# may-/joeys2t

Measured on AMD Instinct MI355X. Metric: audio frames/sec (train step, 80-mel, 15 s utt, bs32 per GPU), higher is better.
Workload: dtype bf16; 1 GPU; configs/librispeech_100h.yaml ASR train step on synthetic 16 kHz waveforms; global_batch=32, frames_per_utt=1498, encoder_len=375, lengths=fixed 15 s, vocab=5000, batch_multiplier=1, parallelism=dp1, launch=hipGraph replay

## Files before the change

### include/joeys2t_hip.h

```cpp
#ifndef JOEYS2T_HIP_H
#define JOEYS2T_HIP_H

#include <stdint.h>

#ifdef __cplusplus
extern "C" {
#endif

typedef void* js2t_stream;

enum { JS2T_F32 = 0, JS2T_BF16 = 1, JS2T_FP8_E4M3 = 2  };
enum { JS2T_ACT_NONE = 0, JS2T_ACT_RELU = 1, JS2T_ACT_GELU = 2, JS2T_ACT_SWISH = 3, JS2T_ACT_TANH = 4, JS2T_ACT_HARDSWISH = 5 };
enum { JS2T_OK = 0, JS2T_ERR_INVALID = -1, JS2T_ERR_LAUNCH = -2, JS2T_ERR_UNSUPPORTED = -3 };

int js2t_abi_version(void);
const char* js2t_last_error(void);

typedef struct js2t_gemm_desc {
  int32_t M, N, K;
  int32_t batch, batch_inner;
  int32_t dtype_ab, dtype_c;
  int32_t trans_a, trans_b;
  const void* A; int64_t lda, a_stride_o, a_stride_i;
  const void* B; int64_t ldb, b_stride_o, b_stride_i;
// ... 8 lines not shown
  uint32_t rng_stream;
  const void* residual;
  int64_t ldr;
  float res_scale;
  const void* gate;
  int64_t ldg;
  float gate_scale;
  float beta;
  int32_t conv, conv_tin, conv_tout, conv_c, conv_stride, conv_pad;
  int32_t split_k;
  float* a_rowsum;
  const float* ln_partial;
  float ln_eps;
  float* ln_mean;
  float* ln_rstd;
  float* rs_partial;
  uint8_t* c8;
  int64_t ldc8;
  float* c8_state;
  const float* c8_mul;
  float* c8_scale_out;
  float* fp8_state;
  const void* dot_src;
  int64_t ld_dot;
  float* dot_partial;
  float* sumsq_partial;
} js2t_gemm_desc;

int js2t_gemm(const js2t_gemm_desc* d, js2t_stream stream);
#define JS2T_GEMM_GROUP_MAX 32
int js2t_gemm_grouped(const js2t_gemm_desc* d, int32_t count, const void* const* A, const void* const* B, void* const* C,
                      float* const* a_rowsum, js2t_stream stream);
int64_t js2t_gemm_grouped_blocks(int32_t M, int32_t N, int32_t count);
void js2t_gemm_force_regstage(int on);
void js2t_gemm_force_w256(int on);
void js2t_gemm_p192_mode(int mode);
void js2t_gemm_wg256_mode(int mode);
void js2t_gemm_p192_ring(int nst);
void js2t_gemm_panel_mode(int mode);


int js2t_axpby(const void* x, float a, const void* y, float b, void* out, int64_t n, int dt, js2t_stream stream);

int js2t_cast(const void* src, int src_dt, void* dst, int dst_dt, int64_t n, js2t_stream stream);

int js2t_fold_ln_weights(const int64_t* table, int32_t n_entries, int32_t max_rows, js2t_stream stream);

int js2t_absmax(const void* x, int dt, int64_t n, float* out, js2t_stream stream);
int js2t_quantize_fp8(const void* x, int dt, void* y, int64_t n, const float* amax, const float* mul, float* scale_out,
                      js2t_stream stream);
int js2t_quantize_fp8_delayed(const void* x, int dt, void* y, int64_t n, float* state, const float* mul, float* scale_out,
                              js2t_stream stream);

int js2t_glu_fwd(const void* x, void* y, int64_t rows, int64_t C, int dt, js2t_stream stream);
int js2t_glu_bwd(const void* x, const void* dy, void* dx, int64_t rows, int64_t C, int dt, js2t_stream stream);
int js2t_glu_fwd_crop(const void* x, void* y, int64_t rows, int64_t C, int64_t T, const int64_t* valid_t, int dt, js2t_stream stream);
int js2t_glu_bwd_crop(const void* x, const void* dy, void* dx, int64_t rows, int64_t C, int64_t T, const int64_t* valid_t, int dt,
                      js2t_stream stream);

int js2t_transpose_groups(const void* src, void* dst, const int64_t* table, int32_t n_groups, int64_t total_tiles, js2t_stream stream);

int js2t_add_pe_dropout(const void* x, const float* pe, const void* extra, void* y, int64_t B, int64_t T,
                        int64_t D, int dt, float p, const uint64_t* rng_state, uint32_t rng_stream,
                        js2t_stream stream);

int js2t_dropout_bwd(const void* dy, void* dx, int64_t rows, int64_t cols, int dt, float p,
// ... 302 lines not shown
```

### joeys2t_amd/csrc/gemm.hip

```cpp
#include "gemm_shared.hpp"
#include <type_traits>

namespace {

bool g_force_regstage = false;
bool g_force_w256 = false;

__device__ __forceinline__ bool a_elem_offset(const js2t_gemm_desc& d, int slow, int fast, int64_t& off) {
  if (!d.conv) {
    off = (int64_t)slow * d.lda + fast;
    return true;
  }
  const int b = slow / d.conv_tout, t = slow - b * d.conv_tout;
  const int kw = fast / d.conv_c;
  const int tin = t * d.conv_stride - d.conv_pad + kw;
  off = ((int64_t)b * d.conv_tin + (t * d.conv_stride - d.conv_pad)) * d.conv_c + fast;
  return tin >= 0 && tin < d.conv_tin;
}

__device__ __forceinline__ void gemm_epilogue4(const js2t_gemm_desc& d, int z, int64_t c_boff, int m, int n,
                                               f32x4_t acc, float alpha) {
  if (m >= d.M || n >= d.N) return;
  const int nv = min(4, d.N - n);
  float v[4];
#pragma unroll
  for (int i = 0; i < 4; ++i) v[i] = acc[i] * alpha;

  if (d.bias) {
#pragma unroll
    for (int i = 0; i < 4; ++i)
      if (i < nv) v[i] += d.bias[n + i];
  }
  const int64_t coff = c_boff + (int64_t)m * d.ldc + n;
// ... 888 lines not shown
      if (do_rs) {
#pragma unroll
        for (int i = 0; i < MI; ++i) racc[i] = __builtin_amdgcn_mfma_f32_16x16x32_bf16(ones, fm[i], racc[i], 0, 0, 0);
      }
    }
    cur = cur + 1 == NST ? 0 : cur + 1;
  }
  if (do_rs && (lane >> 4) == 0) {
    typedef __attribute__((address_space(1))) float gfloat;
#pragma unroll
    for (int i = 0; i < MI; ++i) {
      const int m = m0 + wm * (BM / 2) + 16 * i + lane;
      if (m < M) __builtin_amdgcn_global_atomic_fadd_f32((gfloat*)d.a_rowsum + m, racc[i][0]);
    }
  }
  if constexpr (!SPLITK && !TB) {
    if (direct_tile_epilogue<BM>(d, acc, z, co, m0, n0)) return;
  }
  dma_tile_epilogue<BM, SPLITK, !TB>(d, acc, smem, z, co, m0, n0, c_atomic);
}

template <int BM, bool TA, bool TB, bool SPLITK, int NST = 2>
__global__ __launch_bounds__(256, 2) void gemm_bf16_dma_kernel(js2t_gemm_desc d, int tiles_m, int tiles_n, float* c_atomic,
                                                               int split_k) {
  dma_gemm_block<BM, TA, TB, SPLITK, NST>(d, tiles_m, tiles_n, c_atomic, split_k, blockIdx.y, xcd_remap(blockIdx.x, tiles_m * tiles_n),
                                          blockIdx.z);
}

struct GemmGroup {
  const void* A[JS2T_GEMM_GROUP_MAX];
  const void* B[JS2T_GEMM_GROUP_MAX];
  void* C[JS2T_GEMM_GROUP_MAX];
  float* rowsum[JS2T_GEMM_GROUP_MAX];
};
template <int BM, bool TA, bool TB, bool SPLITK>
__global__ __launch_bounds__(256, 2) void gemm_bf16_dma_grouped_kernel(js2t_gemm_desc d, GemmGroup grp, int tiles_m, int tiles_n,
                                                                       int split_k) {
  const int tiles = tiles_m * tiles_n, nsplit = SPLITK ? split_k : 1;
  const int lid_all = xcd_remap(blockIdx.x, gridDim.x);
  const int vm = lid_all / tiles, tile = lid_all - vm * tiles;
  const int g = vm / nsplit, slice = vm - g * nsplit;
  js2t_gemm_desc dd = d;
  dd.A = grp.A[g];
  dd.B = grp.B[g];
  dd.C = grp.C[g];
  dd.a_rowsum = grp.rowsum[g];
  dma_gemm_block<BM, TA, TB, SPLITK>(dd, tiles_m, tiles_n, (float*)dd.C, split_k, 0, tile, slice);
}

__device__ const uint4 g_zero16 = {0u, 0u, 0u, 0u};
constexpr int W_HALF = 16384;
constexpr int W_LDS = 8 * W_HALF;

__device__ __forceinline__ bf16x8_t w256_frag(const unsigned char* img, int row, int kk, int lane) {
  const int c = kk * 4 + (lane >> 4);
  return *(const bf16x8_t*)(img + row * 128 + ((c ^ (row & 7)) << 4));
}

__global__ __launch_bounds__(512, 1) void gemm_bf16_w256_kernel(js2t_gemm_desc d, int tiles_m, int tiles_n) {
  extern __shared__ __attribute__((aligned(16))) unsigned char smem[];
  const int t = threadIdx.x, lane = t & 63, w = t >> 6, g = lane >> 4;
  const int wr = w >> 2, wc = w & 3;
  const int lid = xcd_remap(blockIdx.x, tiles_m * tiles_n);
  const int m0 = (lid / tiles_n) * 256, n0 = (lid % tiles_n) * 256;
  const int M = d.M, N = d.N, K = d.K;
  const int nk = (K + 63) >> 6;
// ... 1242 lines not shown
        if (m < M) {
          float* crow = Cb + (int64_t)m * d.ldc + tn0 + r;
          float old[8];
          if (beta != 0.f) {
#pragma unroll
            for (int j = 0; j < 8; ++j) old[j] = crow[16 * j];
          }
#pragma unroll
          for (int j = 0; j < 8; ++j) crow[16 * j] = beta != 0.f ? acc[i][j][e] * alpha + beta * old[j] : acc[i][j][e] * alpha;
        }
      }
    }
    if (RS && do_rs && r == 0) {
      typedef __attribute__((address_space(1))) float gfloat;
#pragma unroll
      for (int i = 0; i < 3; ++i)
#pragma unroll
        for (int e = 0; e < 4; ++e) {
          const int m = tm0 + 16 * (w + 4 * i) + 4 * g + e;
          if (m < M) __builtin_amdgcn_global_atomic_fadd_f32((gfloat*)grp.rowsum[mem] + m, racc[i][e]);
        }
    }
  }
  P192_T(6);
  asm volatile("s_waitcnt vmcnt(0)" ::: "memory");
#ifdef JS2T_P192_PROF
  if (blockIdx.x == 0 && t == 0)
    for (int i = 0; i < 8; ++i) g_p192_prof[i] = prof_[i];
#endif
}

constexpr int WG_IMG = 16384, WG_STAGE = 3 * WG_IMG, WG_NST = 3, WG_LDS = WG_NST * WG_STAGE, WG_PER = 12;

template <bool RS, bool SPLITK>
__global__ __launch_bounds__(768, 1) void gemm_bf16_wg256_kernel(js2t_gemm_desc d, GemmGroup grp, int tiles_m, int tiles_n, int split_k) {
  extern __shared__ __attribute__((aligned(16))) unsigned char smem[];
  const int t = threadIdx.x, lane = t & 63;
  const int w = __builtin_amdgcn_readfirstlane(t >> 6);
  const int tiles = tiles_m * tiles_n;
  const int lid = xcd_remap(blockIdx.x, gridDim.x);
  const int vm = lid / tiles, tile = lid - vm * tiles;
  const int mem = SPLITK ? vm / split_k : vm, slice = SPLITK ? vm - mem * split_k : 0;
  const int m0 = (tile / tiles_n) * 256, n0 = (tile % tiles_n) * 128;
  const int K = d.K, nk_all = (K + 63) >> 6;
  const int per = SPLITK ? (nk_all + split_k - 1) / split_k : nk_all;
  const int kt0 = slice * per;
  const int nk = min(per, nk_all - kt0);
  float ss = 0.f;

  if (w >= 8) {
    const int l = w - 8;
    const int64_t lda = d.lda, ldb = d.ldb;
    const uint16_t* zsrc = (const uint16_t*)&g_zero16;
    const uint16_t* src[12];
    int krow[4];
    {
      const uint16_t* Ab = (const uint16_t*)grp.A[mem];
      const uint16_t* Bb = (const uint16_t*)grp.B[mem];
#pragma unroll
      for (int q = 0; q < 4; ++q) {
        const int p = (l * 4 + q) * 64 + lane, kr = p >> 4, col = (((p & 15) ^ (tr_g(kr) << 1)) << 3);
        krow[q] = kr;
        src[q] = Ab + (int64_t)kr * lda + m0 + col;
        src[4 + q] = Ab + (int64_t)kr * lda + m0 + 128 + col;
        src[8 + q] = Bb + (int64_t)kr * ldb + n0 + col;
      }
    }
    auto issue_stage = [&](int st, int slot) {
      const int k0 = st < nk ? (kt0 + st) << 6 : 0;
      const int64_t ka = (int64_t)k0 * lda, kb = (int64_t)k0 * ldb;
      const int klim = K - k0;
      unsigned char* stp = smem + slot * WG_STAGE + l * 4096;
#pragma unroll
      for (int q = 0; q < 12; ++q) {
        const uint16_t* sp = src[q] + (q < 8 ? ka : kb);
        if (klim < 64) {
          if (krow[q & 3] >= klim) sp = zsrc;
        }
        lds_dma16(sp, stp + (q >> 2) * WG_IMG + (q & 3) * 1024);
      }
    };
    issue_stage(0, 0);
    issue_stage(1, 1);
    asm volatile("s_waitcnt vmcnt(%0)" ::"n"(WG_PER) : "memory");
    __builtin_amdgcn_s_barrier();
    asm volatile("" ::: "memory");
    issue_stage(2, 2);
    int cslot = 0;
#ifdef JS2T_P192_PROF
    unsigned long long prof_[8] = {0, 0, 0, 0, 0, 0, 0, 0}, last_ = __builtin_readcyclecounter();
#endif
    for (int s = 0; s < nk; ++s) {
      asm volatile("s_waitcnt vmcnt(%0)" ::"n"(WG_PER) : "memory");
      P192_T(4);
      __builtin_amdgcn_s_barrier();
      asm volatile("" ::: "memory");
      P192_T(5);
      issue_stage(s + 3, cslot);
      P192_T(6);
      cslot = cslot == WG_NST - 1 ? 0 : cslot + 1;
    }
    asm volatile("s_waitcnt vmcnt(0)" ::: "memory");
#ifdef JS2T_P192_PROF
    if (blockIdx.x == 0 && t == 512)
      for (int i = 4; i < 8; ++i) g_p192_prof[i] = prof_[i];
#endif
  } else {
    const int wm = w >> 1, wn = w & 1;
    const int a_img = (wm >> 1) * WG_IMG, a_sub = (wm & 1) * 64, b_sub = wn * 64;
    bf16x8_t fm0[4], fn0[4], fm1[4], fn1[4];
// ... 47 lines not shown
      P192_T(2);
      __builtin_amdgcn_sched_barrier(0);
      const int nslot = cslot == WG_NST - 1 ? 0 : cslot + 1;
      const unsigned char* nst = smem + nslot * WG_STAGE;
#pragma unroll
      for (int i = 0; i < 4; ++i) {
#pragma unroll
        for (int j = 0; j < 4; ++j) acc[i][j] = __builtin_amdgcn_mfma_f32_16x16x32_bf16(fn1[j], fm1[i], acc[i][j], 0, 0, 0);
        if (i < 2) {
          fn0[2 * i] = frag_load2<true>(nst + 2 * WG_IMG, b_sub + 32 * i, 0, lane);
          fn0[2 * i + 1] = frag_load2<true>(nst + 2 * WG_IMG, b_sub + 32 * i + 16, 0, lane);
        } else {
          fm0[2 * i - 4] = frag_load2<true>(nst + a_img, a_sub + 32 * (i - 2), 0, lane);
          fm0[2 * i - 3] = frag_load2<true>(nst + a_img, a_sub + 32 * (i - 2) + 16, 0, lane);
        }
        __builtin_amdgcn_sched_barrier(0);
      }
      if (RS && do_rs) {
#pragma unroll
        for (int i = 0; i < 4; ++i) racc[i] = __builtin_amdgcn_mfma_f32_16x16x32_bf16(ones, fm1[i], racc[i], 0, 0, 0);
      }
      __builtin_amdgcn_sched_barrier(0);
      P192_T(3);
      cslot = nslot;
    }
#ifdef JS2T_P192_PROF
    if (blockIdx.x == 0 && t == 0)
      for (int i = 0; i < 4; ++i) g_p192_prof[i] = prof_[i];
#endif

    if (RS && do_rs && (lane >> 4) == 0) {
      typedef __attribute__((address_space(1))) float gfloat;
#pragma unroll
      for (int i = 0; i < 4; ++i)
        __builtin_amdgcn_global_atomic_fadd_f32((gfloat*)grp.rowsum[mem] + m0 + wm * 64 + 16 * i + lane, racc[i][0]);
    }
    if constexpr (SPLITK) {
      asm volatile("s_waitcnt lgkmcnt(0)" ::: "memory");
      __syncthreads();
      float* Cs = (float*)smem;
#pragma unroll
      for (int i = 0; i < 4; ++i)
#pragma unroll
        for (int j = 0; j < 4; ++j) {
          const int ml = wm * 64 + 16 * i + (lane & 15), n4 = wn * 16 + 4 * j + (lane >> 4);
          *(f32x4_t*)(Cs + ml * 128 + ((n4 ^ (ml & 7)) << 2)) = acc[i][j];
        }
    } else {
    const float alpha = d.alpha * (d.alpha_dev ? *d.alpha_dev : 1.f), beta = d.beta;
    float* Cb = (float*)grp.C[mem] + (int64_t)(m0 + wm * 64 + (lane & 15)) * d.ldc + n0 + wn * 64 + 4 * (lane >> 4);
#pragma unroll
    for (int i = 0; i < 4; ++i) {
      float* crow = Cb + (int64_t)(16 * i) * d.ldc;
      float4 old[4];
      if (beta != 0.f) {
#pragma unroll
        for (int j = 0; j < 4; ++j) old[j] = *(const float4*)(crow + 16 * j);
      }
#pragma unroll
      for (int j = 0; j < 4; ++j) {
        float4 v = make_float4(acc[i][j][0] * alpha, acc[i][j][1] * alpha, acc[i][j][2] * alpha, acc[i][j][3] * alpha);
        if (beta != 0.f) v.x += beta * old[j].x, v.y += beta * old[j].y, v.z += beta * old[j].z, v.w += beta * old[j].w;
        *(float4*)(crow + 16 * j) = v;
        ss = fmaf(v.x, v.x, fmaf(v.y, v.y, fmaf(v.z, v.z, fmaf(v.w, v.w, ss))));
      }
    }
    }
  }
  if constexpr (SPLITK) {
    if (w >= 8) __syncthreads();
    __syncthreads();
    const float alpha = d.alpha * (d.alpha_dev ? *d.alpha_dev : 1.f);
    const float* Cs = (const float*)smem;
    typedef __attribute__((address_space(1))) float gfloat;
    gfloat* cg = (gfloat*)grp.C[mem] + (int64_t)m0 * d.ldc + n0;
    for (int idx = w; idx < 512; idx += 12) {
      const int ml = idx >> 1, nl = (idx & 1) * 64 + lane;
      const float v = Cs[ml * 128 + ((((nl >> 2) ^ (ml & 7)) << 2) | (nl & 3))];
      __builtin_amdgcn_global_atomic_fadd_f32(cg + (int64_t)ml * d.ldc + nl, v * alpha);
    }
    return;
  }
  if (d.sumsq_partial) {
    ss = block_sum(ss, (float*)smem);
    if (t == 0) d.sumsq_partial[2 * blockIdx.x] = ss, d.sumsq_partial[2 * blockIdx.x + 1] = 0.f;
  }
}

#define g_p192_mode js2t_ctx_value(JS2T_CTX_GEMM_P192_MODE)
inline bool p192_eligible(const js2t_gemm_desc& d) {
  if (g_p192_mode == 0) return false;
  if (d.trans_a || d.trans_b || d.conv || d.split_k > 1 || d.batch != 1 || d.dtype_c != JS2T_BF16) return false;
  if ((d.N & 7) || d.N < 128 || (d.K & 7) || d.K < 192 || d.M < 1) return false;
  if (d.preact || d.beta != 0.f || !(d.act == JS2T_ACT_NONE || d.act == JS2T_ACT_RELU) || (d.residual && d.gate)) return false;
  if (!epilogue_rows_aligned(d)) return false;
  if (g_p192_mode < 0 && (int64_t)cdiv(d.M, P_BM) * (d.N >> 7) < 200) return false;
  return true;
}
#define g_p192_ring js2t_ctx_value(JS2T_CTX_GEMM_P192_RING)
enum P192Form { P192_LOADER_CONSUMER, P192_RING2, P192_RING3 };
inline P192Form p192_form(int tiles, int n_cu, int ring, bool stats_dot, bool fp8, bool c8, bool scaled) {
  const bool few = fp8 ? 2 * tiles < 3 * n_cu : tiles <= n_cu;
  const bool lc = fp8 ? (scaled && ring < 0) || ((scaled || !c8) && (ring == 4 || (ring < 0 && few)))
                      : ring == 4 || stats_dot || (ring < 0 && few);
  if (lc) return P192_LOADER_CONSUMER;
  return (ring == 2 || (ring < 0 && !few)) ? P192_RING2 : P192_RING3;
}
template <int EPI, bool FP8 = false>
int launch_p192_epi(const js2t_gemm_desc& d, hipStream_t s) {
  JS2T_LDS_ONCE((gemm_bf16_p192_kernel<EPI, 3, FP8>), P_LDS);
  JS2T_LDS_ONCE((gemm_bf16_p192_kernel<EPI, 2, FP8>), 2 * P_STAGE);
  JS2T_LDS_ONCE((gemm_bf16_p192s_kernel<EPI, FP8>), PS_LDS);
  const int n_cu = js2t_cu_count8();
  if (n_cu <= 0) return JS2T_ERR_LAUNCH;
  const int tm = cdiv(d.M, P_BM), tn = cdiv(d.N, 128), tiles = tm * tn;
  const int one = tiles < n_cu ? tiles : n_cu, two = tiles < 2 * n_cu ? tiles : 2 * n_cu;
  switch (p192_form(tiles, n_cu, g_p192_ring, EPI >= 0 && (EPI & (PE_STATS | PE_DOT)), FP8, d.c8 != nullptr, P192S_SCALED)) {
    case P192_LOADER_CONSUMER: hipLaunchKernelGGL((gemm_bf16_p192s_kernel<EPI, FP8>), dim3(one), dim3(768), PS_LDS, s, d, tm, tn); break;
// ... 167 lines not shown
    for (int i = 0; i < count; ++i) JS2T_CHECK(aligned(C[i]), "gemm_grouped: sumsq_partial needs 16-byte aligned C");
  }
  for (int base = 0; base < count; base += JS2T_GEMM_GROUP_MAX) {
    const int n = count - base < JS2T_GEMM_GROUP_MAX ? count - base : JS2T_GEMM_GROUP_MAX;
    GemmGroup grp;
    for (int i = 0; i < JS2T_GEMM_GROUP_MAX; ++i) {
      const int j = base + (i < n ? i : 0);
      JS2T_CHECK(A[j] && B[j] && C[j] && aligned(A[j]) && aligned(B[j]), "gemm_grouped: operands must be non-null, 16-byte aligned");
      grp.A[i] = A[j], grp.B[i] = B[j], grp.C[i] = C[j];
      grp.rowsum[i] = a_rowsum ? a_rowsum[j] : nullptr;
    }
    d.A = grp.A[0], d.B = grp.B[0], d.C = grp.C[0];
    int rc;
    bool c16 = true;
    for (int i = 0; i < n; ++i) c16 = c16 && aligned(grp.C[i]);
    if (c16 && wg256_eligible(d, n)) {
      if (d.split_k > 1)
        rc = a_rowsum ? launch_grouped_wg256<true, true>(d, grp, n, (hipStream_t)stream) : launch_grouped_wg256<false, true>(d, grp, n, (hipStream_t)stream);
      else
        rc = a_rowsum ? launch_grouped_wg256<true, false>(d, grp, n, (hipStream_t)stream) : launch_grouped_wg256<false, false>(d, grp, n, (hipStream_t)stream);
    } else if (!d.sumsq_partial && p192t_eligible(d, n)) {
      rc = a_rowsum ? launch_grouped_p192t<true>(d, grp, n, (hipStream_t)stream) : launch_grouped_p192t<false>(d, grp, n, (hipStream_t)stream);
    } else {
      rc = d.split_k > 1 ? launch_grouped_tt<true>(d, grp, n, (hipStream_t)stream) : launch_grouped_tt<false>(d, grp, n, (hipStream_t)stream);
    }
    if (rc != JS2T_OK) return rc;
    if (d.sumsq_partial) d.sumsq_partial += (int64_t)cdiv(d.M, 128) * cdiv(d.N, F_BN) * n;
  }
  return JS2T_OK;
}

extern "C" int64_t js2t_gemm_grouped_blocks(int32_t M, int32_t N, int32_t count) {
  return (int64_t)cdiv(M, 128) * cdiv(N, F_BN) * count;
}

extern "C" int js2t_gemm(const js2t_gemm_desc* dp, js2t_stream stream) {
  JS2T_CHECK(dp != nullptr, "gemm: null descriptor");
  js2t_gemm_desc d = *dp;
  JS2T_CHECK(!d.sumsq_partial, "gemm: sumsq_partial is taken by js2t_gemm_grouped only");
  hipStream_t s = (hipStream_t)stream;
  JS2T_CHECK(d.M >= 0 && d.N >= 0 && d.K >= 0 && d.batch >= 0, "gemm: negative size");
  if (d.M == 0 || d.N == 0 || d.batch == 0) return JS2T_OK;
  JS2T_CHECK(d.A && d.B && (d.C || (d.c8 && d.dtype_ab == JS2T_FP8_E4M3)), "gemm: null operand");
  JS2T_CHECK(!d.c8 || (d.dtype_ab == JS2T_FP8_E4M3 && d.c8_state && d.ldc8 >= d.N && (d.ldc8 & 7) == 0 && aligned(d.c8, 8) &&
                       aligned(d.c8_state)),
             "gemm: c8 (e4m3 second output) needs e4m3 operands, c8_state (16-byte aligned) and 8-byte aligned rows");
  JS2T_CHECK(d.batch_inner >= 1, "gemm: batch_inner must be >= 1");
  JS2T_CHECK(d.dtype_ab == JS2T_F32 || d.dtype_ab == JS2T_BF16 || d.dtype_ab == JS2T_FP8_E4M3, "gemm: bad dtype_ab");
  JS2T_CHECK(d.dtype_c == JS2T_F32 || d.dtype_c == JS2T_BF16, "gemm: bad dtype_c");
  JS2T_CHECK(d.dropout_p >= 0.f && d.dropout_p < 1.f, "gemm: dropout_p out of range");
  JS2T_CHECK(d.dropout_p == 0.f || d.rng_state, "gemm: dropout needs rng_state");
  JS2T_CHECK(!d.residual || d.ldr > 0, "gemm: residual needs ldr");
  JS2T_CHECK(!d.gate || d.ldg > 0, "gemm: gate needs ldg");
  JS2T_CHECK(d.batch <= 65535, "gemm: batch too large");
  if (d.conv) {
    JS2T_CHECK(d.conv_c > 0 && d.conv_tin > 0 && d.conv_tout > 0 && d.conv_stride > 0, "gemm: bad conv geometry");
  }
  JS2T_CHECK(!(d.residual || d.gate) || d.batch == 1, "gemm: residual / gate need batch == 1");
  JS2T_CHECK(!d.a_rowsum || (d.batch == 1 && !d.conv && !g_force_regstage && d.trans_a && d.trans_b),
             "gemm: a_rowsum needs trans_a = trans_b = 1, batch == 1 and the LDS-DMA kernel");
  if (d.split_k < 1) d.split_k = 1;
  if (d.split_k > 1) {
    JS2T_CHECK(d.dtype_c == JS2T_F32 && !d.bias && d.act == JS2T_ACT_NONE && !d.preact && d.dropout_p == 0.f && !d.residual &&
                   !d.gate && d.beta == 0.f,
               "gemm: split_k needs an f32 C and a plain epilogue (C must be zero-filled by the caller)");
    if (g_js2t_deterministic) d.split_k = 1, d.beta = 1.f;
// ... 53 lines not shown
```

### joeys2t_amd/ops.py

```python
import ctypes as C
import math
from typing import Optional, Sequence

import torch

from joeys2t_amd._lib import ACT_CODES, BF16, F32, AttnDesc, GemmDesc, Js2tError, check, lib

FP8 = 2
_DT = {torch.float32: F32, torch.bfloat16: BF16, torch.float8_e4m3fn: FP8}


def dt_code(t_or_dtype) -> int:
    dtype = t_or_dtype.dtype if torch.is_tensor(t_or_dtype) else t_or_dtype
    try:
        return _DT[dtype]
    except KeyError:
        raise Js2tError(f"unsupported dtype {dtype}: the HIP path computes in float32 or bfloat16") from None


def _dev(*tensors):
    for t in tensors:
        if t is not None and not t.is_cuda:
            raise Js2tError(
                "joeys2t_amd ops run on the GPU through libjoeys2t_hip.so only; got a CPU tensor "
# ... 168 lines not shown
    n = len(As)
    if not (n == len(Bs) == len(Cs)) or (a_rowsums is not None and len(a_rowsums) != n):
        raise Js2tError("gemm_grouped: list lengths differ")
    if n == 0:
        return
    _dev(*As, *Bs, *Cs, *(a_rowsums or ()))
    if any(t.dtype != torch.bfloat16 for t in (*As, *Bs)) or any(c.dtype != Cs[0].dtype for c in Cs):
        raise Js2tError("gemm_grouped: bf16 operands and one output dtype required")
    d = GemmDesc()
    d.M, d.N, d.K = int(M), int(N), int(K)
    d.batch, d.batch_inner = 1, 1
    d.dtype_ab, d.dtype_c = BF16, dt_code(Cs[0])
    d.trans_a, d.trans_b = 1, 1
    d.lda, d.ldb, d.ldc = int(lda), int(ldb), int(ldc)
    d.alpha, d.beta, d.split_k = float(alpha), float(beta), int(split_k)
    d.res_scale = d.gate_scale = 1.0
    if sumsq_partial is not None:
        _dev(sumsq_partial)
        if sumsq_partial.dtype != torch.float32 or sumsq_partial.numel() < grouped_blocks(d.M, d.N, n):
            raise Js2tError("gemm_grouped: sumsq_partial must be f32[grouped_blocks(M, N, count)]")
        d.sumsq_partial = sumsq_partial.data_ptr()
    arr = C.c_void_p * n
    pa, pb, pc = arr(*[t.data_ptr() for t in As]), arr(*[t.data_ptr() for t in Bs]), arr(*[t.data_ptr() for t in Cs])
    pr = None if a_rowsums is None else arr(*[t.data_ptr() for t in a_rowsums])
    if GEMM_TIMER is not None:
        GEMM_TIMER.wrap(f"js2t_gemm_grouped<split_k {'>' if d.split_k > 1 else '='} 1> (gemm_bf16_wg256_kernel | gemm_bf16_dma_grouped_kernel)",
                        2.0 * d.M * d.N * d.K * n,
                        lambda: check(lib().js2t_gemm_grouped(C.byref(d), n, pa, pb, pc, pr, _stream()), "js2t_gemm_grouped"),
                        nbytes=n * (2 * (d.M * d.K + d.N * d.K) + Cs[0].element_size() * d.M * d.N * (2 if d.beta else 1)))
    else:
        check(lib().js2t_gemm_grouped(C.byref(d), n, pa, pb, pc, pr, _stream()), "js2t_gemm_grouped")


def grouped_blocks(M: int, N: int, count: int) -> int:
    return lib().js2t_gemm_grouped_blocks(M, N, count)


def cast(src: torch.Tensor, dtype: torch.dtype, out: Optional[torch.Tensor] = None) -> torch.Tensor:
    _dev(src, out)
    src = src.contiguous()
    if out is None:
        out = torch.empty(src.shape, dtype=dtype, device=src.device)
    check(lib().js2t_cast(_p(src), dt_code(src), _p(out), dt_code(out), src.numel(), _stream()), "js2t_cast")
    return out


def axpby(x, a: float, y=None, b: float = 0.0):
    _dev(x, y)
    out = torch.empty_like(x)
    check(lib().js2t_axpby(_p(x), a, _p(y), b, _p(out), x.numel(), dt_code(x), _stream()), "js2t_axpby")
    return out


def transpose_groups(src, dst, table, n_groups: int, total_tiles: int):
    _dev(src, dst, table)
    check(lib().js2t_transpose_groups(_p(src), _p(dst), _p(table), n_groups, total_tiles, _stream()), "js2t_transpose_groups")


def glu_fwd(x: torch.Tensor, T: Optional[int] = None, valid_t: Optional[torch.Tensor] = None) -> torch.Tensor:
    _dev(x, valid_t)
    rows, c2 = x.shape[0], x.shape[1]
    y = torch.empty((rows, c2 // 2), dtype=x.dtype, device=x.device)
    check(lib().js2t_glu_fwd_crop(_p(x), _p(y), rows, c2 // 2, T if valid_t is not None else max(rows, 1), _p(valid_t), dt_code(x),
                                  _stream()), "js2t_glu_fwd")
    return y

# ... 1071 lines not shown
```

### joeys2t_amd/runtime.py

```python
from typing import Dict, List, Optional, Sequence, Tuple

import torch
from torch import nn

from joeys2t_amd import ops

_ALIGN = 64


class ParamStore:

    def __init__(self, module: nn.Module, device: torch.device):
        self.device = torch.device(device)
        group_of: Dict[int, List[nn.Parameter]] = {}
        for m in module.modules():
            fg = getattr(m, "fuse_groups", None)
            if fg is None:
                continue
            for grp in fg():
                grp = [p for p in grp if p is not None]
                if any(id(p) in group_of for p in grp):
                    continue
                for p in grp:
                    group_of[id(p)] = grp
        groups: List[List[nn.Parameter]] = []
        seen = set()
        for p in module.parameters():
            if id(p) in seen:
                continue
            grp = group_of.get(id(p), [p])
            for q in grp:
                seen.add(id(q))
# ... 259 lines not shown
        if active:
            for _, items in plan:
                for it in items:
                    seen[it[2].data_ptr()] = seen.get(it[2].data_ptr(), 0) + 1
        for key, items in plan:
            mode = 0
            if active:
                N, K, M = key[:3]
                spans = [self._span(it[2]) for it in items]
                solo = all(seen[it[2].data_ptr()] == 1 and it[2].is_contiguous() and it[2].dtype == torch.float32 for it in items)
                unsplit = wgrad_split(N, K, M, count=len(items)) == 1 and wgrad_split(N, K, 1 << 30, count=len(items)) == 1
                if solo and unsplit and all(cand.contains(*s) for s in spans):
                    if self.first:
                        mode |= 1
                        written.extend(spans)
                    if self.collector is not None and K % 128 == 0:
                        mode |= 2
            out.append((key + (mode, self.collector if mode & 2 else None), items))
        if active and self.first:
            written = self._written + written
            self._written = [] if final else written
            if final:
                for lo, hi in self.kept.minus(written):
                    self.grad_base[lo:hi].zero_()
                    self.kept.remove(lo, hi)
            for lo, hi in written:
                if not self.kept.contains(lo, hi):
                    self.kept.add(lo, hi)
        return out

    @staticmethod
    def run(plan, on_group_done=None):
        from joeys2t_amd.functional import wgrad_split
        for key, items in plan:
            N, K, M, lda, ldb, has_db = key[:6]
            mode, collector = (key[6], key[7]) if len(key) > 6 else (0, None)
            n = len(items)
            sk = wgrad_split(N, K, M, count=n)
            part = None
            if mode & 2:
                lo = [(it[2].data_ptr() - collector.grad.data_ptr()) // 4 for it in items]
                part = collector.segment(ops.grouped_blocks(N, K, n), [(a, a + it[2].numel()) for a, it in zip(lo, items)])
            ops.gemm_grouped([it[0] for it in items], [it[1] for it in items], [it[2] for it in items], M=N, N=K, K=M, lda=lda,
                             ldb=ldb, ldc=K, split_k=sk, beta=0.0 if (sk > 1 or mode & 1) else 1.0,
                             a_rowsums=[it[3] for it in items] if has_db else None, sumsq_partial=part)
            if on_group_done is not None:
                on_group_done(items)


class RangeSet:

    def __init__(self, ranges=()):
        self.r: List[Tuple[int, int]] = []
        for lo, hi in sorted(ranges):
            if self.r and lo <= self.r[-1][1]:
                self.r[-1] = (self.r[-1][0], max(hi, self.r[-1][1]))
            elif hi > lo:
                self.r.append((lo, hi))
        self.version = 0

    def contains(self, lo: int, hi: int) -> bool:
        return any(a <= lo and hi <= b for a, b in self.r)

    def minus(self, spans) -> List[Tuple[int, int]]:
        out = []
        cut = RangeSet(spans).r
        for a, b in self.r:
            pos = a
            for lo, hi in cut:
                if hi <= pos or lo >= b:
                    continue
                if lo > pos:
                    out.append((pos, lo))
                pos = max(pos, hi)
            if pos < b:
                out.append((pos, b))
        return out

    def remove(self, lo: int, hi: int):
        self.r = RangeSet(self.minus([(lo, hi)])).r
# ... 116 lines not shown
```

Before: 4.199 million frames/s.

## Merge compatible wgrad grouped GEMMs of differing M into one wg256 launch

Adds a mixed-shape grouped GEMM entry point that runs weight-gradient products with different M (and lda, beta, sumsq segment) in one 256x128 wg256 launch. A per-member tile_end table maps blocks to members, and partial M tiles are zero-filled and masked. On the host, members are bin-packed across the 8 XCDs. The runtime greedily merges wgrad groups that share K, token count and ldb whenever the merged wave count is lower than running them separately. This targets tail-wave underutilization and per-launch overhead in the backward weight-gradient phase. The cost is added tile lookup and masking work in the kernel, and merged groups lose split-K.

```diff
diff --git a/include/joeys2t_hip.h b/include/joeys2t_hip.h
--- a/include/joeys2t_hip.h
+++ b/include/joeys2t_hip.h
@@ -64,6 +64,9 @@
 int js2t_gemm_grouped(const js2t_gemm_desc* d, int32_t count, const void* const* A, const void* const* B, void* const* C,
                       float* const* a_rowsum, js2t_stream stream);
 int64_t js2t_gemm_grouped_blocks(int32_t M, int32_t N, int32_t count);
+int js2t_gemm_grouped_mixed(const js2t_gemm_desc* d, int32_t count, const void* const* A, const void* const* B, void* const* C,
+                            float* const* a_rowsum, const int32_t* M, const int64_t* lda, const float* beta,
+                            float* const* sumsq_partial, js2t_stream stream);
 void js2t_gemm_force_regstage(int on);
 void js2t_gemm_force_w256(int on);
 void js2t_gemm_p192_mode(int mode);
diff --git a/joeys2t_amd/csrc/gemm.hip b/joeys2t_amd/csrc/gemm.hip
--- a/joeys2t_amd/csrc/gemm.hip
+++ b/joeys2t_amd/csrc/gemm.hip
@@ -1,4 +1,5 @@
 #include "gemm_shared.hpp"
+#include <algorithm>
 #include <type_traits>
 
 namespace {
@@ -953,6 +954,11 @@
   const void* B[JS2T_GEMM_GROUP_MAX];
   void* C[JS2T_GEMM_GROUP_MAX];
   float* rowsum[JS2T_GEMM_GROUP_MAX];
+  float* sumsq[JS2T_GEMM_GROUP_MAX];
+  int64_t lda[JS2T_GEMM_GROUP_MAX];
+  int M[JS2T_GEMM_GROUP_MAX];
+  float beta[JS2T_GEMM_GROUP_MAX];
+  int tile_end[JS2T_GEMM_GROUP_MAX];
 };
 template <int BM, bool TA, bool TB, bool SPLITK>
 __global__ __launch_bounds__(256, 2) void gemm_bf16_dma_grouped_kernel(js2t_gemm_desc d, GemmGroup grp, int tiles_m, int tiles_n,
@@ -2261,15 +2267,24 @@
 
 constexpr int WG_IMG = 16384, WG_STAGE = 3 * WG_IMG, WG_NST = 3, WG_LDS = WG_NST * WG_STAGE, WG_PER = 12;
 
-template <bool RS, bool SPLITK>
+template <bool RS, bool SPLITK, bool MIXED = false>
 __global__ __launch_bounds__(768, 1) void gemm_bf16_wg256_kernel(js2t_gemm_desc d, GemmGroup grp, int tiles_m, int tiles_n, int split_k) {
+  static_assert(!(SPLITK && MIXED), "a mixed launch is never K-split");
   extern __shared__ __attribute__((aligned(16))) unsigned char smem[];
   const int t = threadIdx.x, lane = t & 63;
   const int w = __builtin_amdgcn_readfirstlane(t >> 6);
   const int tiles = tiles_m * tiles_n;
   const int lid = xcd_remap(blockIdx.x, gridDim.x);
-  const int vm = lid / tiles, tile = lid - vm * tiles;
+  int vm, tile;
+  if constexpr (MIXED) {
+    vm = 0;
+    while (vm < JS2T_GEMM_GROUP_MAX - 1 && lid >= grp.tile_end[vm]) ++vm;
+    tile = lid - (vm ? grp.tile_end[vm - 1] : 0);
+  } else {
+    vm = lid / tiles, tile = lid - vm * tiles;
+  }
   const int mem = SPLITK ? vm / split_k : vm, slice = SPLITK ? vm - mem * split_k : 0;
+  const int Mi = MIXED ? grp.M[mem] : 0;
   const int m0 = (tile / tiles_n) * 256, n0 = (tile % tiles_n) * 128;
   const int K = d.K, nk_all = (K + 63) >> 6;
   const int per = SPLITK ? (nk_all + split_k - 1) / split_k : nk_all;
@@ -2279,10 +2294,12 @@
 
   if (w >= 8) {
     const int l = w - 8;
-    const int64_t lda = d.lda, ldb = d.ldb;
+    const int64_t lda = MIXED ? grp.lda[mem] : d.lda, ldb = d.ldb;
     const uint16_t* zsrc = (const uint16_t*)&g_zero16;
     const uint16_t* src[12];
     int krow[4];
+    const bool part_m = MIXED && m0 + 256 > Mi;
+    unsigned zcol = 0;
     {
       const uint16_t* Ab = (const uint16_t*)grp.A[mem];
       const uint16_t* Bb = (const uint16_t*)grp.B[mem];
@@ -2293,6 +2310,7 @@
         src[q] = Ab + (int64_t)kr * lda + m0 + col;
         src[4 + q] = Ab + (int64_t)kr * lda + m0 + 128 + col;
         src[8 + q] = Bb + (int64_t)kr * ldb + n0 + col;
+        if constexpr (MIXED) zcol |= (m0 + col >= Mi ? 1u << q : 0u) | (m0 + 128 + col >= Mi ? 16u << q : 0u);
       }
     }
     auto issue_stage = [&](int st, int slot) {
@@ -2305,6 +2323,11 @@
         const uint16_t* sp = src[q] + (q < 8 ? ka : kb);
         if (klim < 64) {
           if (krow[q & 3] >= klim) sp = zsrc;
+        }
+        if constexpr (MIXED) {
+          if (q < 8 && part_m) {
+            if ((zcol >> q) & 1) sp = zsrc;
+          }
         }
         lds_dma16(sp, stp + (q >> 2) * WG_IMG + (q & 3) * 1024);
       }
@@ -2418,8 +2441,10 @@
     if (RS && do_rs && (lane >> 4) == 0) {
       typedef __attribute__((address_space(1))) float gfloat;
 #pragma unroll
-      for (int i = 0; i < 4; ++i)
-        __builtin_amdgcn_global_atomic_fadd_f32((gfloat*)grp.rowsum[mem] + m0 + wm * 64 + 16 * i + lane, racc[i][0]);
+      for (int i = 0; i < 4; ++i) {
+        const int m = m0 + wm * 64 + 16 * i + lane;
+        if (!MIXED || m < Mi) __builtin_amdgcn_global_atomic_fadd_f32((gfloat*)grp.rowsum[mem] + m, racc[i][0]);
+      }
     }
     if constexpr (SPLITK) {
       asm volatile("s_waitcnt lgkmcnt(0)" ::: "memory");
@@ -2433,10 +2458,12 @@
           *(f32x4_t*)(Cs + ml * 128 + ((n4 ^ (ml & 7)) << 2)) = acc[i][j];
         }
     } else {
-    const float alpha = d.alpha * (d.alpha_dev ? *d.alpha_dev : 1.f), beta = d.beta;
-    float* Cb = (float*)grp.C[mem] + (int64_t)(m0 + wm * 64 + (lane & 15)) * d.ldc + n0 + wn * 64 + 4 * (lane >> 4);
+    const float alpha = d.alpha * (d.alpha_dev ? *d.alpha_dev : 1.f), beta = MIXED ? grp.beta[mem] : d.beta;
+    const int mrow = m0 + wm * 64 + (lane & 15);
+    float* Cb = (float*)grp.C[mem] + (int64_t)mrow * d.ldc + n0 + wn * 64 + 4 * (lane >> 4);
 #pragma unroll
     for (int i = 0; i < 4; ++i) {
+      if (MIXED && mrow + 16 * i >= Mi) continue;
       float* crow = Cb + (int64_t)(16 * i) * d.ldc;
       float4 old[4];
       if (beta != 0.f) {
@@ -2467,9 +2494,11 @@
     }
     return;
   }
-  if (d.sumsq_partial) {
+  float* ssp = MIXED ? grp.sumsq[mem] : d.sumsq_partial;
+  if (ssp) {
     ss = block_sum(ss, (float*)smem);
-    if (t == 0) d.sumsq_partial[2 * blockIdx.x] = ss, d.sumsq_partial[2 * blockIdx.x + 1] = 0.f;
+    ssp += 2 * (int64_t)(MIXED ? tile : (int)blockIdx.x);
+    if (t == 0) ssp[0] = ss, ssp[1] = 0.f;
   }
 }
 
@@ -2703,6 +2732,97 @@
 
 extern "C" int64_t js2t_gemm_grouped_blocks(int32_t M, int32_t N, int32_t count) {
   return (int64_t)cdiv(M, 128) * cdiv(N, F_BN) * count;
+}
+
+template <bool RS>
+static int launch_grouped_wg256_mixed(const js2t_gemm_desc& d, const GemmGroup& grp, int total, hipStream_t s) {
+  JS2T_LDS_ONCE((gemm_bf16_wg256_kernel<RS, false, true>), WG_LDS);
+  hipLaunchKernelGGL((gemm_bf16_wg256_kernel<RS, false, true>), dim3(total), dim3(768), WG_LDS, s, d, grp, 0, d.N >> 7, 1);
+  JS2T_LAUNCH_CHECK();
+  return JS2T_OK;
+}
+
+extern "C" int js2t_gemm_grouped_mixed(const js2t_gemm_desc* dp, int32_t count, const void* const* A, const void* const* B, void* const* C,
+                                       float* const* a_rowsum, const int32_t* M, const int64_t* lda, const float* beta,
+                                       float* const* sumsq_partial, js2t_stream stream) {
+  JS2T_CHECK(dp != nullptr && count >= 0, "gemm_grouped_mixed: bad arguments");
+  if (count == 0) return JS2T_OK;
+  JS2T_CHECK(A && B && C && M && lda && beta, "gemm_grouped_mixed: null tables");
+  const js2t_gemm_desc& d = *dp;
+  JS2T_CHECK(d.N > 0 && d.K > 0, "gemm_grouped_mixed: empty product");
+  JS2T_CHECK(d.dtype_ab == JS2T_BF16 && d.trans_a && d.trans_b && !d.conv && d.batch == 1,
+             "gemm_grouped_mixed: bf16 reduction-major operands only (trans_a = trans_b = 1, batch = 1)");
+  JS2T_CHECK(!d.bias && d.act == JS2T_ACT_NONE && !d.preact && d.dropout_p == 0.f && !d.residual && !d.gate && !d.alpha_dev,
+             "gemm_grouped_mixed: plain epilogue only (alpha, beta_i)");
+  JS2T_CHECK(!d.sumsq_partial, "gemm_grouped_mixed: partial sums go to the members' own segments (sumsq_partial[i])");
+#define JS2T_MIXED_NEEDS(cond, text)                          \
+  do {                                                        \
+    if (!(cond)) {                                            \
+      js2t_set_error("gemm_grouped_mixed: needs %s", text);  \
+      return JS2T_ERR_UNSUPPORTED;                            \
+    }                                                         \
+  } while (0)
+  JS2T_MIXED_NEEDS(count <= JS2T_GEMM_GROUP_MAX, "at most JS2T_GEMM_GROUP_MAX members");
+  JS2T_MIXED_NEEDS(g_wg256_mode != 0 && d.split_k <= 1 && d.dtype_c == JS2T_F32, "the 256x128 kernel, un-split, f32 C");
+  JS2T_MIXED_NEEDS((d.N & 127) == 0 && (d.ldc & 3) == 0 && d.ldc >= d.N && (d.ldb & 7) == 0 && d.ldb >= d.N && d.K >= 192,
+                   "N % 128 == 0, 16-byte rows of B and C, K >= 192");
+  GemmGroup grp = {};
+  const int tn = d.N >> 7;
+  int tiles[JS2T_GEMM_GROUP_MAX];
+  int64_t total = 0;
+  for (int i = 0; i < count; ++i) {
+    JS2T_MIXED_NEEDS(M[i] > 0 && (M[i] & 7) == 0 && (lda[i] & 7) == 0 && lda[i] >= M[i], "M_i % 8 == 0, lda_i % 8 == 0, lda_i >= M_i");
+    JS2T_MIXED_NEEDS(beta[i] == 0.f || beta[i] == 1.f, "beta_i of 0 or 1");
+    JS2T_MIXED_NEEDS(A[i] && B[i] && C[i] && aligned(A[i]) && aligned(B[i]) && aligned(C[i]), "non-null, 16-byte aligned operands and C");
+    JS2T_MIXED_NEEDS(!(sumsq_partial && sumsq_partial[i]) || (cdiv(M[i], 128) & 1) == 0, "an even number of 128-row tiles where sums of squares are asked for");
+    tiles[i] = cdiv(M[i], 256) * tn;
+    total += tiles[i];
+  }
+  JS2T_MIXED_NEEDS(total < (1 << 30), "fewer tiles");
+  if (g_wg256_mode < 0) JS2T_MIXED_NEEDS(d.K >= 1024 && total >= 160, "(automatic rule) >= 160 tiles over K >= 1024");
+#undef JS2T_MIXED_NEEDS
+  int order[JS2T_GEMM_GROUP_MAX], bin_of[JS2T_GEMM_GROUP_MAX], load[8] = {0, 0, 0, 0, 0, 0, 0, 0};
+  for (int i = 0; i < count; ++i) order[i] = i;
+  std::stable_sort(order, order + count, [&](int a, int b) { return tiles[a] > tiles[b]; });
+  for (int k = 0; k < count; ++k) {
+    int best = 0;
+    for (int x = 1; x < 8; ++x)
+      if (load[x] < load[best]) best = x;
+    bin_of[order[k]] = best, load[best] += tiles[order[k]];
+  }
+  const int n_cu = js2t_cu_count8();
+  if (n_cu <= 0) return JS2T_ERR_LAUNCH;
+  const int per_round = n_cu >= 8 ? n_cu / 8 : 1;
+  int slot = 0, end = 0;
+  for (int x = 0; x < 8; ++x) {
+    bool used[JS2T_GEMM_GROUP_MAX] = {};
+    for (int room = per_round;;) {
+      int pick = -1, largest = -1;
+      for (int k = 0; k < count; ++k) {
+        const int i = order[k];
+        if (bin_of[i] != x || used[i]) continue;
+        if (largest < 0) largest = i;
+        if (tiles[i] <= room) {
+          pick = i;
+          break;
+        }
+      }
+      if (largest < 0) break;
+      const int i = pick >= 0 ? pick : largest;
+      used[i] = true;
+      room = per_round - (per_round - room + tiles[i]) % per_round;
+      grp.A[slot] = A[i], grp.B[slot] = B[i], grp.C[slot] = C[i];
+      grp.rowsum[slot] = a_rowsum ? a_rowsum[i] : nullptr;
+      grp.sumsq[slot] = sumsq_partial ? sumsq_partial[i] : nullptr;
+      grp.lda[slot] = lda[i], grp.M[slot] = M[i], grp.beta[slot] = beta[i];
+      grp.tile_end[slot++] = end += tiles[i];
+    }
+  }
+  for (; slot < JS2T_GEMM_GROUP_MAX; ++slot) grp.tile_end[slot] = end;
+  js2t_gemm_desc dd = d;
+  dd.split_k = 1, dd.A = grp.A[0], dd.B = grp.B[0], dd.C = grp.C[0];
+  return a_rowsum ? launch_grouped_wg256_mixed<true>(dd, grp, end, (hipStream_t)stream)
+                  : launch_grouped_wg256_mixed<false>(dd, grp, end, (hipStream_t)stream);
 }
 
 extern "C" int js2t_gemm(const js2t_gemm_desc* dp, js2t_stream stream) {
diff --git a/joeys2t_amd/ops.py b/joeys2t_amd/ops.py
--- a/joeys2t_amd/ops.py
+++ b/joeys2t_amd/ops.py
@@ -224,6 +224,59 @@
         check(lib().js2t_gemm_grouped(C.byref(d), n, pa, pb, pc, pr, _stream()), "js2t_gemm_grouped")
 
 
+GROUP_MAX = 32
+
+
+class _MixedUnsupported(Exception):
+    pass
+
+
+def gemm_grouped_mixed(As, Bs, Cs, *, Ms, N, K, ldas, ldb, ldc, betas, alpha=1.0, a_rowsums=None, sumsq_partials=None) -> bool:
+    n = len(As)
+    if not (n == len(Bs) == len(Cs) == len(Ms) == len(ldas) == len(betas)) or (a_rowsums is not None and len(a_rowsums) != n) or (
+            sumsq_partials is not None and len(sumsq_partials) != n):
+        raise Js2tError("gemm_grouped_mixed: list lengths differ")
+    if n == 0:
+        return True
+    parts = [p for p in (sumsq_partials or ()) if p is not None]
+    _dev(*As, *Bs, *Cs, *(a_rowsums or ()), *parts)
+    if any(t.dtype != torch.bfloat16 for t in (*As, *Bs)) or any(c.dtype != torch.float32 for c in Cs):
+        raise Js2tError("gemm_grouped_mixed: bf16 operands and f32 outputs required")
+    d = GemmDesc()
+    d.N, d.K = int(N), int(K)
+    d.batch, d.batch_inner = 1, 1
+    d.dtype_ab, d.dtype_c = BF16, F32
+    d.trans_a, d.trans_b = 1, 1
+    d.ldb, d.ldc = int(ldb), int(ldc)
+    d.alpha, d.split_k = float(alpha), 1
+    d.res_scale = d.gate_scale = 1.0
+    if sumsq_partials is not None:
+        for p, m in zip(sumsq_partials, Ms):
+            if p is not None and (p.dtype != torch.float32 or not p.is_contiguous() or p.numel() < grouped_blocks(int(m), d.N, 1)):
+                raise Js2tError("gemm_grouped_mixed: sumsq_partials[i] must be contiguous f32[grouped_blocks(M_i, N, 1)]")
+    arr = C.c_void_p * n
+    pa, pb, pc = arr(*[t.data_ptr() for t in As]), arr(*[t.data_ptr() for t in Bs]), arr(*[t.data_ptr() for t in Cs])
+    pr = None if a_rowsums is None else arr(*[t.data_ptr() for t in a_rowsums])
+    ps = None if sumsq_partials is None else arr(*[None if p is None else p.data_ptr() for p in sumsq_partials])
+    pm, pl, pbeta = (C.c_int32 * n)(*map(int, Ms)), (C.c_int64 * n)(*map(int, ldas)), (C.c_float * n)(*map(float, betas))
+
+    def launch():
+        rc = lib().js2t_gemm_grouped_mixed(C.byref(d), n, pa, pb, pc, pr, pm, pl, pbeta, ps, _stream())
+        if rc == -3:
+            raise _MixedUnsupported()
+        check(rc, "js2t_gemm_grouped_mixed")
+
+    try:
+        if GEMM_TIMER is not None:
+            GEMM_TIMER.wrap("js2t_gemm_grouped_mixed (gemm_bf16_wg256_kernel)", 2.0 * sum(map(int, Ms)) * d.N * d.K, launch,
+                            nbytes=sum(2 * (int(m) * d.K + d.N * d.K) + 4 * int(m) * d.N * (2 if b else 1) for m, b in zip(Ms, betas)))
+        else:
+            launch()
+    except _MixedUnsupported:
+        return False
+    return True
+
+
 def grouped_blocks(M: int, N: int, count: int) -> int:
     return lib().js2t_gemm_grouped_blocks(M, N, count)
 
diff --git a/joeys2t_amd/runtime.py b/joeys2t_amd/runtime.py
--- a/joeys2t_amd/runtime.py
+++ b/joeys2t_amd/runtime.py
@@ -1,3 +1,4 @@
+import os
 from typing import Dict, List, Optional, Sequence, Tuple
 
 import torch
@@ -323,20 +324,89 @@
     @staticmethod
     def run(plan, on_group_done=None):
         from joeys2t_amd.functional import wgrad_split
+        todo = []
         for key, items in plan:
             N, K, M, lda, ldb, has_db = key[:6]
             mode, collector = (key[6], key[7]) if len(key) > 6 else (0, None)
             n = len(items)
-            sk = wgrad_split(N, K, M, count=n)
             part = None
             if mode & 2:
                 lo = [(it[2].data_ptr() - collector.grad.data_ptr()) // 4 for it in items]
                 part = collector.segment(ops.grouped_blocks(N, K, n), [(a, a + it[2].numel()) for a, it in zip(lo, items)])
-            ops.gemm_grouped([it[0] for it in items], [it[1] for it in items], [it[2] for it in items], M=N, N=K, K=M, lda=lda,
-                             ldb=ldb, ldc=K, split_k=sk, beta=0.0 if (sk > 1 or mode & 1) else 1.0,
-                             a_rowsums=[it[3] for it in items] if has_db else None, sumsq_partial=part)
+            todo.append((N, K, M, lda, ldb, has_db, mode, part, wgrad_split(N, K, M, count=n), items))
+        sets = [[i] for i in range(len(todo))]
+        if WGRAD_MERGE and len(todo) > 1:
+            sets = wgrad_merge_sets([_merge_desc(t) for t in todo], _cu_count(todo[0][9][0][0].device), ops.GROUP_MAX)
+        first = {s[0]: s for s in sets}
+        launched = [False] * len(todo)
+        for i, (N, K, M, lda, ldb, has_db, mode, part, sk, items) in enumerate(todo):
+            if not launched[i] and len(first.get(i, ())) > 1 and _run_merged([todo[j] for j in first[i]]):
+                for j in first[i]:
+                    launched[j] = True
+            if not launched[i]:
+                ops.gemm_grouped([it[0] for it in items], [it[1] for it in items], [it[2] for it in items], M=N, N=K, K=M, lda=lda,
+                                 ldb=ldb, ldc=K, split_k=sk, beta=0.0 if (sk > 1 or mode & 1) else 1.0,
+                                 a_rowsums=[it[3] for it in items] if has_db else None, sumsq_partial=part)
+                launched[i] = True
             if on_group_done is not None:
                 on_group_done(items)
+
+
+WGRAD_MERGE = os.environ.get("JS2T_WGRAD_MERGE", "1") != "0"
+WGRAD_MERGE_MIN_TOKENS = int(os.environ.get("JS2T_WGRAD_MERGE_MIN_TOKENS", "8192"))
+_CU_COUNT: Dict[torch.device, int] = {}
+
+
+def _cu_count(device) -> int:
+    if device not in _CU_COUNT:
+        _CU_COUNT[device] = torch.cuda.get_device_properties(device).multi_processor_count if device.type == "cuda" else 0
+    return _CU_COUNT[device]
+
+
+def _merge_desc(t):
+    N, K, M, lda, ldb, has_db, mode, part, sk, items = t
+    dw = [it[2] for it in items]
+    ok = (M >= max(WGRAD_MERGE_MIN_TOKENS, 192) and N % 8 == 0 and K % 128 == 0 and lda % 8 == 0 and
+          all(w.dtype == torch.float32 and w.is_contiguous() for w in dw))
+    return ((K, M, ldb, has_db, dw[0].dtype) if ok else None, len(items) * (-(-N // 256)) * (K // 128), len(items), sk > 1)
+
+
+def wgrad_merge_sets(groups, n_cu: int, max_members: int):
+    if n_cu <= 0:
+        return [[i] for i in range(len(groups))]
+    rounds = lambda tiles, split: 1 if split else -(-tiles // n_cu)
+    taken, out = [False] * len(groups), []
+    for i, (key, tiles, members, split) in enumerate(groups):
+        if taken[i]:
+            continue
+        taken[i] = True
+        cur, cost = [i], rounds(tiles, split)
+        if key is not None:
+            for j in range(i + 1, len(groups)):
+                kj, tj, mj, sj = groups[j]
+                if taken[j] or kj != key or members + mj > max_members:
+                    continue
+                merged = -(-(tiles + tj) // n_cu)
+                if merged < cost + rounds(tj, sj):
+                    taken[j] = True
+                    cur.append(j)
+                    tiles, members, cost = tiles + tj, members + mj, merged
+        out.append(cur)
+    return out
+
+
+def _run_merged(entries) -> bool:
+    As, Bs, Cs, Ms, ldas, betas, rows, parts = [], [], [], [], [], [], [], []
+    N0, K, M, lda0, ldb, has_db = entries[0][:6]
+    for N, _, _, lda, _, _, mode, part, sk, items in entries:
+        per = ops.grouped_blocks(N, K, 1) if part is not None else 0
+        for k, it in enumerate(items):
+            As.append(it[0]), Bs.append(it[1]), Cs.append(it[2]), rows.append(it[3])
+            Ms.append(N), ldas.append(lda)
+            betas.append(0.0 if (sk == 1 and mode & 1) else 1.0)
+            parts.append(part[k * per:(k + 1) * per] if part is not None else None)
+    return ops.gemm_grouped_mixed(As, Bs, Cs, Ms=Ms, N=K, K=M, ldas=ldas, ldb=ldb, ldc=K, betas=betas,
+                                  a_rowsums=rows if has_db else None, sumsq_partials=parts if any(p is not None for p in parts) else None)
 
 
 class RangeSet:
```

After: 4.230 million frames/s (median of 6 runs). No clear change (+0.7%).
